# pyannote/pyannote-video

Measured on AMD Instinct MI355X. Metric: frames/sec end-to-end detect->embed->cluster, 1080p@25fps, higher is better.
Workload: dtype f32 (detector scores, embedder) / f64 (tracker, clustering) / u8 frames; an f16 screening pass with a proven error bound decides which windows the detector's exact f32 chain is evaluated for -- results identical to dense f32 scoring (`dense_scoring`)

## Files before the change

pyannote-video_amd/csrc/api.hip:

```cpp
#include "pvf_internal.h"
#include <algorithm>
#include <cmath>
#include <cstdlib>
#include <string>
#include <thread>

#define API_BEGIN try {
#define API_END                                                        \
    return 0;                                                          \
    }                                                                  \
    catch (const std::exception& e) { pvf_set_error(e.what()); return -1; } \
    catch (...) { pvf_set_error("unknown error"); return -2; }

#define ENTER(c, h)                                                \
    Ctx* c = pvf_ctx(h);                                           \
    std::lock_guard<std::recursive_mutex> _api_lock(c->api_mu);    \
    HIP_CHECK(hipSetDevice(c->device))
#define ENTER_DET(c, h)                                            \
    Ctx* c = pvf_ctx(h);                                           \
    std::lock_guard<std::recursive_mutex> _det_lock(c->det_mu);    \
    HIP_CHECK(hipSetDevice(c->device))
#define ENTER_BOTH(c, h)                                           \
    Ctx* c = pvf_ctx(h);                                           \
    std::lock_guard<std::recursive_mutex> _det_lock(c->det_mu);    \
// ... 829 lines not shown
        const size_t bytes = (size_t)n * 150 * 150 * 3;
        c->s_trk0.ensure(bytes);
        HIP_CHECK(hipMemcpyAsync(c->s_trk0.p, chips, bytes, hipMemcpyHostToDevice, c->stream));
    }
    resnet_debug_stage(c, c->s_trk0.as<uint8_t>(), n, split != 0, &tap, flags);
    for (int i = 0; i < 3; ++i) dims[i] = tap.dims[i];
    API_END
}

extern "C" int32_t pvf_debug_conv(pvf_handle h, const int32_t geom[18], const float* in, const float* w, const float* bias, const float* gamma,
                                  const float* beta, const float* skip, int32_t split, int32_t force_generic, float* out, int32_t* flags)
{
    API_BEGIN
    ENTER(c, h);
    PVF_REQUIRE(geom, "pvf_debug_conv: bad arguments");
    resnet_debug_conv(c, geom, in, w, bias, gamma, beta, skip, split != 0, force_generic != 0, out, flags);
    API_END
}

extern "C" int32_t pvf_debug_embed_head(pvf_handle h, const float* x, int32_t n, int32_t hw, float* out)
{
    API_BEGIN
    ENTER(c, h);
    resnet_debug_head(c, x, n, hw, out);
    API_END
}

static PairInput table_f64(const double* X) { PairInput in; in.X = X; return in; }
static PairOutput host_full(double* D) { PairOutput o; o.out = D; return o; }

extern "C" int32_t pvf_pair_mean_dist(pvf_handle h, const double* X, int32_t N, int32_t dim, const int32_t* row_start, int32_t T, double* D)
// ... 374 lines not shown
```

pyannote-video_amd/csrc/ctx.hip:

```cpp
#include "pvf_internal.h"
#include "detect_ml.h"
#include <cmath>
#include <fstream>
#include <mutex>
#include <dlfcn.h>

static thread_local std::string g_err;
void pvf_set_error(const char* msg) { g_err = msg ? msg : ""; }
extern "C" const char* pvf_last_error(void) { return g_err.c_str(); }

static std::mutex g_ctx_mu;
static std::unordered_map<uint64_t, std::unique_ptr<Ctx>> g_ctxs;
static uint64_t g_next_ctx = 0x1000;

Ctx* pvf_ctx(pvf_handle h)
{
    std::lock_guard<std::mutex> lk(g_ctx_mu);
    auto it = g_ctxs.find(h);
    if (it == g_ctxs.end()) throw PvfError("unknown context handle");
    return it->second.get();
}

std::map<std::string, Tensor> pvf_read_container(const char* path)
{
// ... 143 lines not shown
{
    auto m = pvf_read_model(path, 2);
    EmbedModel& e = c->emb;
    e.chip_size = need(m, "emb.meta").i32()[0];
    e.chip_padding = need(m, "emb.padding").f64()[0];
    PVF_REQUIRE(e.chip_size == 150, "embedder: 150x150 chips expected");
    const Tensor& ms = need(m, "emb.mean_shape");
    PVF_REQUIRE(ms.numel() == 102, "emb.mean_shape must be 51x2");
    e.mean_shape.assign(ms.f32(), ms.f32() + 102);
    const Tensor& blob = need(m, "emb.blob");
    const float* p = blob.f32();
    const float* end = p + blob.numel();
    for (ConvLayer& L : e.convs) {
        if (L.d_frag) { (void)hipFree(L.d_frag); L.d_frag = nullptr; }
        if (L.d_wsplit) { (void)hipFree(L.d_wsplit); L.d_wsplit = nullptr; }
    }
    e.convs.clear();
    if (e.d_stem) { (void)hipFree(e.d_stem); e.d_stem = nullptr; }
    auto add_conv = [&](int cin, int cout, int k, int stride, int pad) {
        ConvLayer L{cin, cout, k, stride, pad, nullptr, nullptr, nullptr, nullptr, nullptr};
        const size_t nw = (size_t)cout * cin * k * k;
        PVF_REQUIRE(p + nw + 3 * (size_t)cout <= end, "emb.blob too short");
        conv_layer_upload(L, p, p + nw, p + nw + cout, p + nw + 2 * (size_t)cout);
        p += nw + 3 * (size_t)cout;
        e.convs.push_back(L);
    };
    add_conv(3, 32, 7, 2, 0);
    for (int u = 0; u < 14; ++u) {
        const int cin = UNITS[u][0], n = UNITS[u][1], down = UNITS[u][2];
        add_conv(cin, n, 3, down ? 2 : 1, down ? 0 : 1);
        add_conv(n, n, 3, 1, 1);
    }
// ... 385 lines not shown
```

pyannote-video_amd/csrc/pvf_internal.h:

```cpp
#pragma once
#include <hip/hip_runtime.h>
#include <cstdint>
#include <cstdio>
#include <cstring>
#include <deque>
#include <map>
#include <atomic>
#include <memory>
#include <mutex>
#include <stdexcept>
#include <string>
#include <unordered_map>
#include <vector>
#include "../../include/pvface.h"
#include "scratch_layout.h"
#include "chip_plan.h"

#define PVF_FHOG_STRIDE 32

struct CandOverflow : PvfError { int needed; explicit CandOverflow(int n) : PvfError("detector: candidate buffer overflow"), needed(n) {} };
struct ScreenRetry : PvfError { ScreenRetry() : PvfError("detector: screening pass gave up") {} };

#define HIP_CHECK(expr)                                                                              \
    do {                                                                                             \
// ... 115 lines not shown
    int32_t* d_idx1 = nullptr;
    int32_t* d_idx2 = nullptr;
    float* d_thresh = nullptr;
    float* d_leaves = nullptr;
};

struct ConvLayer {
    int cin, cout, k, stride, pad;
    float* d_w;
    float* d_bias;
    float* d_gamma;
    float* d_beta;
    float* d_frag = nullptr;
    int w_exp = 0;
    uint32_t* d_wsplit = nullptr;
};

struct EmbedModel {
    bool loaded = false;
    int chip_size = 150;
    double chip_padding = 0.25;
    std::vector<float> mean_shape;
    std::vector<ConvLayer> convs;
    float* d_fc = nullptr;
    float* d_blob = nullptr;
    float* d_stem = nullptr;
};

struct TrackerTables {
    bool set = false;
    double* d_mask64 = nullptr;
    double* d_mask_scale = nullptr;
    double* d_tw64 = nullptr;
    double* d_tw32 = nullptr;
    double alpha_pow_m16 = 0, ln_alpha = 0;
};

struct Tracker {
    double* d_state = nullptr;
    int* share = nullptr;
    double pos[4] = {0, 0, 0, 0};
// ... 170 lines not shown
void jitter_embed_dev(Ctx* c, const uint8_t* d_chips, int n, int J, uint64_t seed, float* out);
void ert_run(Ctx* c, const std::vector<Frame>& frames, const pvf_rect_i32* boxes, int n, int32_t* pts, float* shape = nullptr);
void face_chip_details(const EmbedModel& m, const int32_t* pts68, ChipDetails* out);
void dlib_mean_face_shape(float* out );
void resnet_forward(Ctx* c, const uint8_t* d_chips, int n, float* h_out);
struct ChipSource { const uint8_t* host; const pvf_handle* frames; const int32_t* pts; };
const EmbedModel& faces_geometry();
void faces_make_chips(Ctx* c, const pvf_handle* frames, const int32_t* pts, int m, uint8_t* d_chips);
void faces_source_round(Ctx* c, const ChipSource& src, int i0, int m, uint8_t* d_chips);
void conv_layer_upload(ConvLayer& L, const float* w, const float* bias, const float* gamma, const float* beta);
void conv_layer_free(ConvLayer& L);
#define EMB_STAGES 30
struct EmbedTap { int stage; float* h_out; int dims[3]; };
void resnet_debug_stage(Ctx* c, const uint8_t* d_chips, int n, bool split, EmbedTap* tap, int* h_flags);
void resnet_debug_conv(Ctx* c, const int32_t* geom, const float* in, const float* w, const float* bias, const float* gamma, const float* beta,
                       const float* skip, bool split, bool force_generic, float* out, int32_t* flags);
void resnet_debug_head(Ctx* c, const float* x, int n, int hw, float* out);
void dsst_start_many(Ctx* c, const std::vector<Tracker*>& t, const std::vector<Frame>& f, const double* boxes);
void dsst_clone_many(Ctx* c, const std::vector<Tracker*>& src, const std::vector<Tracker*>& dst);
double* tracker_state_alloc(Ctx* c);
void shot_dfd(Ctx* c, const std::vector<Frame>& frames, int ow, int oh, const float* tables22, double* dfd, uint8_t* gray_out, float* flow_out);
std::vector<int> orb_level_quota();
void orb_extract(Ctx* c, const std::vector<Frame>& frames, int ow, int oh, int cap, int32_t* counts, float* kp_out, uint8_t* desc_out);
void orb_match_counts(Ctx* c, const uint8_t* desc, const int32_t* nrows, int n_sets, int cap, const int32_t* pairs, int64_t n_pairs, int32_t* out);
void dsst_update_many(Ctx* c, const std::vector<Tracker*>& t, const std::vector<Frame>& f, double* psr, double* boxes_out, int mode = 0);
void overlap_matrix_host(const double* a, int na, const double* b, int nb, double ratio, double* out);
void munkres_host(const double* cost, int n, int32_t* row_to_col);
struct PairInput {
    const double* X = nullptr;
    const float* emb = nullptr; int64_t emb_stride = 0; int n_src = 0; const int32_t* order = nullptr; int decimals = -1; bool emb_on_device = false;
};
// ... 14 lines not shown
```

pyannote-video_amd/csrc/resnet.hip:

```cpp
#include "pvf_internal.h"
#include <cmath>
#include <cstdlib>
#include <cstring>
#include <vector>

typedef float f32x4 __attribute__((ext_vector_type(4)));
typedef uint32_t u32x4 __attribute__((ext_vector_type(4)));
typedef float f32x16 __attribute__((ext_vector_type(16)));
typedef _Float16 f16x8 __attribute__((ext_vector_type(8)));
typedef _Float16 f16x4 __attribute__((ext_vector_type(4)));
typedef uint32_t u32x2 __attribute__((ext_vector_type(2)));

void face_chip_details(const EmbedModel& m, const int32_t* pts, ChipDetails* out)
{
    const double size = m.chip_size, padding = m.chip_padding;
    double fx[51], fy[51], tx[51], ty[51];
    int n = 0;
    for (int i = 17; i < 68; ++i) {
        if ((55 <= i && i <= 59) || (65 <= i && i <= 67)) continue;
        if (17 <= i && i <= 26) continue;
        fx[n] = ((padding + (double)m.mean_shape[2 * (i - 17)]) / (2 * padding + 1)) * size;
        fy[n] = ((padding + (double)m.mean_shape[2 * (i - 17) + 1]) / (2 * padding + 1)) * size;
        tx[n] = pts[2 * i]; ty[n] = pts[2 * i + 1];
        ++n;
// ... 18 lines not shown
    out->cs = ca / scale; out->sn = cb / scale;
    out->rows = m.chip_size; out->cols = m.chip_size;
}

struct ConvArgs {
    const float* in; int B, H, W, Cin;
    const float* w; int K;
    const float* frag;
    const float* bias; const float* gamma; const float* beta;
    float* out; int OH, OW, Cout;
    int AH, AW;
    int ksz, stride, pad;
    int skip_mode;
    const float* skip; int XH, XW, XC, SH, SW;
    const uint32_t* wsplit; float out_scale; int* flags;
};


__device__ __forceinline__ int small_div(int x, int d, float rd)
{
    int q = (int)((float)x * rd);
    const int r = x - q * d;
    q += (r >= d) ? 1 : 0;
    q -= (r < 0) ? 1 : 0;
    return q;
}

template <int WM, int WN>
__device__ __forceinline__ void conv_epilogue(const ConvArgs& a, float* smem, const f32x16& acc0, const f32x16& acc1, long M, long m0, int n0,
                                              int rel0, int b_first, int hw, float r_hw, float r_ow, int wave, int lane)
// ... 311 lines not shown
        }
    }
    const float bs = bias[li], g = gamma[li], bt = beta[li];
    float* o = out + ((size_t)face * OW + oy0) * OW * 32 + li;
#pragma unroll
    for (int t = 0; t < 3; ++t)
#pragma unroll
        for (int reg = 0; reg < 16; ++reg) {
            const int m = (wave * 3 + t) * 32 + (reg & 3) + 8 * (reg >> 2) + 4 * kh;
            float v = (acc[t][reg] + bs) * g + bt;
            v = v < 0.0f ? 0.0f : v;
            o[(size_t)m * 32] = v;
        }
}

#define C32_ROWS 7
#define C32_TILE_FLOATS (9 * 37 * 33)
__global__ void __launch_bounds__(64) conv_frag_k(const float* __restrict__ w, int Kpad, float* __restrict__ frag)
{
    const int s = blockIdx.x, l = threadIdx.x;
    frag[s * 64 + l] = w[(size_t)(l & 31) * Kpad + 2 * s + (l >> 5)];
}

__global__ void __launch_bounds__(256) conv3x3_c32_k(const float* __restrict__ in, const float* __restrict__ frag, const float* __restrict__ bias,
                                                     const float* __restrict__ gamma, const float* __restrict__ beta, const float* __restrict__ skip,
                                                     float* __restrict__ out, int n_items)
{
    constexpr int HW = 35, TW = 37, PITCH = 33, NP = 144;
    constexpr int NSLOT = 9 * TW * 8, PER = (NSLOT + 255) / 256;
    extern __shared__ __attribute__((aligned(16))) float smem_c32[];
// ... 90 lines not shown
            for (int t = 0; t < 2; ++t)
#pragma unroll
                for (int reg = 0; reg < 16; ++reg) {
                    const float y = ((acc[t][reg] + bs) * g + bt) + sk[t][reg];
                    x[t][reg] = y < 0.0f ? 0.0f : y;
                }
        } else {
#pragma unroll
            for (int t = 0; t < 2; ++t)
#pragma unroll
                for (int reg = 0; reg < 16; ++reg) {
                    const float y = (acc[t][reg] + bs) * g + bt;
                    x[t][reg] = y < 0.0f ? 0.0f : y;
                }
        }
#pragma unroll
        for (int t = 0; t < 2; ++t)
#pragma unroll
            for (int reg = 0; reg < 16; ++reg)
                __builtin_amdgcn_raw_buffer_store_b32(__builtin_bit_cast(uint32_t, x[t][reg]), ro, e_off[t][reg], 0, 0);
        __syncthreads();
        item = next;
    }
}

__global__ void __launch_bounds__(256) maxpool3s2_k(const float* __restrict__ in, int B, int H, int W, int C, float* __restrict__ out, int OH, int OW)
{
    const size_t i = (size_t)blockIdx.x * blockDim.x + threadIdx.x;
    const size_t total = (size_t)B * OH * OW * C;
    if (i >= total) return;
// ... 26 lines not shown
    }
}

static bool conv_is_c32(const ConvArgs& a)
{
    return a.Cin == 32 && a.Cout == 32 && a.H == 35 && a.W == 35 && a.OH == 35 && a.OW == 35 && a.AH == 35 && a.AW == 35 && a.ksz == 3 &&
           a.stride == 1 && a.pad == 1 && a.skip_mode != 2;
}

static void launch_conv(Ctx* c, const ConvArgs& a)
{
    const long M = (long)a.B * a.OH * a.OW;
    PVF_REQUIRE(a.Cin % 32 == 0, "conv: input channels must be a multiple of 32 (the 3-channel first layer has a kernel of its own: stem_conv_k)");
    PVF_REQUIRE(a.OH * a.OW < (1 << 21) && a.Cout % 32 == 0, "conv: output map too large for the kernel's index arithmetic / Cout not a multiple of 32");
    auto tile = [&](auto exact, auto split, dim3 grid) { hipLaunchKernelGGL((a.wsplit ? split : exact), grid, dim3(256), 0, c->stream, a); };
    if (a.frag && conv_is_c32(a)) {
        static std::atomic<uint64_t> attr_set{0};
        const size_t lds = (size_t)(C32_TILE_FLOATS + 144 * 64) * sizeof(float);
        const uint64_t bit = 1ull << (c->device & 63);
        if (!(attr_set.load() & bit)) {
            HIP_CHECK(hipFuncSetAttribute(reinterpret_cast<const void*>(conv3x3_c32_k), hipFuncAttributeMaxDynamicSharedMemorySize, (int)lds));
            attr_set.fetch_or(bit);
        }
        const int items = a.B * (35 / C32_ROWS);
        hipLaunchKernelGGL(conv3x3_c32_k, dim3((unsigned)std::min(items, 2 * c->n_cu)), dim3(256), lds, c->stream, a.in, a.frag, a.bias, a.gamma, a.beta,
                           a.skip_mode == 1 ? a.skip : nullptr, a.out, items);
    } else if (a.Cout == 32) {
        tile(conv_tile_k<4, 1, ConvExact>, conv_tile_k<4, 1, ConvSplit>, dim3((unsigned)((M + 255) / 256), 1));
    } else {
        PVF_REQUIRE(a.Cout % 64 == 0, "conv: Cout must be 32 or a multiple of 64");
        tile(conv_tile_k<2, 2, ConvExact>, conv_tile_k<2, 2, ConvSplit>, dim3((unsigned)((M + 127) / 128), a.Cout / 64));
// ... 19 lines not shown
        HIP_CHECK(hipMemcpy(d, src, count * sizeof(float), hipMemcpyHostToDevice));
        return d;
    };
    L.d_w = up(wt.data(), wt.size());
    float wmax = 0.0f;
    for (float v : wt) wmax = std::max(wmax, std::fabs(v));
    int ex = 0;
    if (wmax > 0.0f && std::isfinite(wmax)) { std::frexp(wmax, &ex); L.w_exp = 15 - ex; }
    L.d_bias = up(bias, cout);
    L.d_gamma = up(gamma, cout);
    L.d_beta = up(beta, cout);
}

void conv_layer_free(ConvLayer& L)
{
    for (void* p : {(void*)L.d_w, (void*)L.d_bias, (void*)L.d_gamma, (void*)L.d_beta, (void*)L.d_frag, (void*)L.d_wsplit})
        if (p) (void)hipFree(p);
    L.d_w = L.d_bias = L.d_gamma = L.d_beta = L.d_frag = nullptr;
    L.d_wsplit = nullptr;
}

static void conv_bind_weights(Ctx* c, ConvLayer& L, bool split, bool generic, int* flags, ConvArgs& a)
{
    a.w = L.d_w; a.K = L.k * L.k * L.cin; a.bias = L.d_bias; a.gamma = L.d_gamma; a.beta = L.d_beta;
    a.frag = nullptr; a.wsplit = nullptr; a.out_scale = 0.0f; a.flags = nullptr;
    if (!generic && L.cin == 32 && L.cout == 32 && L.k == 3) {
        if (!conv_is_c32(a)) return;
        if (!L.d_frag) {
            HIP_CHECK(hipMalloc(&L.d_frag, 144 * 64 * sizeof(float)));
            hipLaunchKernelGGL(conv_frag_k, dim3(144), dim3(64), 0, c->stream, L.d_w, 288, L.d_frag);
        }
        a.frag = L.d_frag;
        return;
    }
    if (!split) return;
    if (!L.d_wsplit) {
        const int Kpad = (L.k * L.k * L.cin + 31) / 32 * 32;
        const int total = L.cout * Kpad;
        HIP_CHECK(hipMalloc(&L.d_wsplit, (size_t)total * 2 * sizeof(_Float16)));
        hipLaunchKernelGGL(conv_wsplit_k, dim3((unsigned)((total + 255) / 256)), dim3(256), 0, c->stream, L.d_w, total, L.w_exp,
                           reinterpret_cast<_Float16*>(L.d_wsplit));
    }
// ... 92 lines not shown
    c->s_act1.ensure(big * sizeof(float));
    c->s_act2.ensure((size_t)cap * hp * hp * 32 * sizeof(float) + (size_t)cap * 128 * sizeof(float));
    PVF_REQUIRE(!tap || n <= MAXB, "embedder stage access: at most 4096 faces");
    auto tapped = [&](int stage, const float* d, int B, int H, int W, int C) {
        if (tap && tap->stage == stage && tap->h_out)
            HIP_CHECK(hipMemcpyAsync(tap->h_out, d, (size_t)B * H * W * C * sizeof(float), hipMemcpyDeviceToHost, c->stream));
    };
    for (int b0 = 0; b0 < n; b0 += MAXB) {
        const int B = std::min(MAXB, n - b0);
        ProfScope ps(c, "conv");
        float* x = c->s_act0.as<float>();
        float* y = c->s_act1.as<float>();
        float* z = c->s_act2.as<float>();
        const ConvLayer& L0 = e.convs[0];
        PVF_REQUIRE(S == 150 && L0.cout == 32 && L0.k == 7 && h1 == 72, "stem kernel: 150 x 150 chips, 7 x 7 stride 2, 32 channels");
        if (!c->emb.d_stem) {
            HIP_CHECK(hipMalloc(&c->emb.d_stem, STEM_NP * 64 * sizeof(float)));
            hipLaunchKernelGGL(stem_frag_k, dim3(STEM_NP), dim3(64), 0, c->stream, L0.d_w, c->emb.d_stem);
        }
        hipLaunchKernelGGL(stem_conv_k, dim3(h1 / STEM_ROWS, B), dim3(192), 0, c->stream, d_chips + (size_t)b0 * S * S * 3, B, c->emb.d_stem,
                           L0.d_bias, L0.d_gamma, L0.d_beta, y);
        tapped(0, y, B, h1, h1, 32);
        ConvArgs a;
        const size_t npool = (size_t)B * hp * hp * 32;
        hipLaunchKernelGGL(maxpool3s2_k, dim3((unsigned)((npool + 255) / 256)), dim3(256), 0, c->stream, y, B, h1, h1, 32, z, hp, hp);
        tapped(1, z, B, hp, hp, 32);
        float* cur = z; float* t1 = x; float* t2 = y;
        int H = hp;
        int* flags = nullptr;
        if (split) {
            flags = c->s_emb_flags.as<int>();
            HIP_CHECK(hipMemsetAsync(flags, 0, (size_t)B * sizeof(int), c->stream));
        }
        for (int u = 0; u < 14; ++u) {
            const int cin = UN[u][0], nn = UN[u][1], down = UN[u][2];
            ConvLayer& La = c->emb.convs[1 + 2 * u];
            ConvLayer& Lb = c->emb.convs[2 + 2 * u];
            const int stride = down ? 2 : 1, pad = down ? 0 : 1;
            const auto [ah, sh, oh] = unit_dims(u, H);
            memset(&a, 0, sizeof a);
            a.in = cur; a.B = B; a.H = H; a.W = H; a.Cin = cin;
            a.out = t1; a.OH = ah; a.OW = ah; a.Cout = nn; a.AH = ah; a.AW = ah; a.ksz = 3; a.stride = stride; a.pad = pad; a.skip_mode = 0;
            conv_bind_weights(c, La, split, false, flags, a);
            launch_conv(c, a);
            tapped(2 + 2 * u, t1, B, ah, ah, nn);
            memset(&a, 0, sizeof a);
            a.in = t1; a.B = B; a.H = ah; a.W = ah; a.Cin = nn;
            a.out = t2; a.OH = oh; a.OW = oh; a.Cout = nn; a.AH = ah; a.AW = ah; a.ksz = 3; a.stride = 1; a.pad = 1;
            a.skip_mode = down ? 2 : 1; a.skip = cur; a.XH = H; a.XW = H; a.XC = cin; a.SH = sh; a.SW = sh;
            conv_bind_weights(c, Lb, split, false, flags, a);
            launch_conv(c, a);
            tapped(3 + 2 * u, t2, B, oh, oh, nn);
            float* old = cur; cur = t2; t2 = old;
            H = oh;
        }
        float* d_out = reinterpret_cast<float*>(c->s_act2.as<uint8_t>() + (size_t)cap * hp * hp * 32 * sizeof(float));
        hipLaunchKernelGGL(head_k, dim3(B), dim3(256), 0, c->stream, cur, H * H, e.d_fc, d_out);
        HIP_CHECK(hipGetLastError());
        HIP_CHECK(hipMemcpyAsync(h_out + (size_t)b0 * 128, d_out, (size_t)B * 128 * sizeof(float), hipMemcpyDeviceToHost, c->stream));
        if (split) HIP_CHECK(hipMemcpyAsync(h_flags + b0, flags, (size_t)B * sizeof(int), hipMemcpyDeviceToHost, c->stream));
    }
    HIP_CHECK(hipStreamSynchronize(c->stream));
}

void resnet_forward(Ctx* c, const uint8_t* d_chips, int n, float* h_out)
// ... 43 lines not shown
struct Scoped {
    void* p = nullptr;
    explicit Scoped(size_t bytes) { HIP_CHECK(hipMalloc(&p, bytes ? bytes : 4)); }
    ~Scoped() { if (p) (void)hipFree(p); }
    Scoped(const Scoped&) = delete;
    Scoped& operator=(const Scoped&) = delete;
};
struct ScopedLayer {
    ConvLayer L{};
    ~ScopedLayer() { conv_layer_free(L); }
};
struct Drain { Ctx* c; ~Drain() { (void)hipStreamSynchronize(c->stream); } };
}

void resnet_debug_conv(Ctx* c, const int32_t* g, const float* in, const float* w, const float* bias, const float* gamma, const float* beta,
                       const float* skip, bool split, bool force_generic, float* out, int32_t* flags)
{
    ConvArgs a;
    memset(&a, 0, sizeof a);
    a.B = g[0]; a.H = g[1]; a.W = g[2]; a.Cin = g[3]; a.OH = g[4]; a.OW = g[5]; a.Cout = g[6]; a.AH = g[7]; a.AW = g[8];
    a.ksz = g[9]; a.stride = g[10]; a.pad = g[11]; a.skip_mode = g[12]; a.XH = g[13]; a.XW = g[14]; a.XC = g[15]; a.SH = g[16]; a.SW = g[17];
    PVF_REQUIRE(in && w && bias && gamma && beta && out, "pvf_debug_conv: null tensor");
    PVF_REQUIRE(a.B > 0 && a.H > 0 && a.W > 0 && a.Cin > 0 && a.OH > 0 && a.OW > 0 && a.Cout > 0 && a.ksz > 0 && a.ksz <= 7 && a.stride > 0 && a.pad >= 0,
                "pvf_debug_conv: bad dimensions");
    PVF_REQUIRE(a.AH > 0 && a.AW > 0 && a.AH <= a.OH && a.AW <= a.OW, "pvf_debug_conv: the convolution's extent must lie inside the output map");
    PVF_REQUIRE(a.skip_mode >= 0 && a.skip_mode <= 2 && (a.skip_mode == 0 || skip), "pvf_debug_conv: skip_mode must be 0..2, with a skip tensor for 1 and 2");
    const size_t n_in = (size_t)a.B * a.H * a.W * a.Cin, n_out = (size_t)a.B * a.OH * a.OW * a.Cout;
    size_t n_skip = 0;
    if (a.skip_mode == 1) n_skip = n_out;
    if (a.skip_mode == 2) {
        PVF_REQUIRE(a.XH > 0 && a.XW > 0 && a.XC > 0 && a.SH >= 0 && a.SW >= 0 && 2 * a.SH <= a.XH && 2 * a.SW <= a.XW,
                    "pvf_debug_conv: the averaged skip map must lie inside the skip tensor");
        n_skip = (size_t)a.B * a.XH * a.XW * a.XC;
    }
    PVF_REQUIRE(n_in < (1u << 30) && n_out < (1u << 30) && n_skip < (1u << 30), "pvf_debug_conv: tensor too large");
    ScopedLayer sl;
    sl.L.cin = a.Cin; sl.L.cout = a.Cout; sl.L.k = a.ksz; sl.L.stride = a.stride; sl.L.pad = a.pad;
// ... 39 lines not shown
```

pyannote-video_amd/pyannote_video_amd/runtime.py:

```python
import contextlib
import ctypes as C
import threading
import itertools
import operator
import numpy as np
from . import _lib
from ._lib import check, ptr, handles
from . import models as _models
from .y4m import YuvFrame, chroma_shape


class DeviceFrame(object):
    __slots__ = ("ctx", "handle", "height", "width", "keep", "transient", "__weakref__")

    def __init__(self, ctx, handle, height, width, keep=None, transient=False):
        self.ctx, self.handle, self.height, self.width, self.keep = ctx, handle, height, width, keep
        self.transient = transient

    @property
    def shape(self):
        return (self.height, self.width, 3)

    def release(self):
        if self.handle is not None and self.ctx._h is not None:
# ... 789 lines not shown
        if skip_mode == 2:
            _, xh, xw, xc = skip.shape
            sh, sw = xh // 2, xw // 2
        oh, ow = out_hw if out_hw is not None else (max(ah, sh), max(aw, sw))
        if skip_mode == 1 and skip.shape != (B, oh, ow, cout):
            raise ValueError("debug_conv: the skip tensor must have the output's shape")
        if skip_mode == 2 and skip.shape[0] != B:
            raise ValueError("debug_conv: one skip map per face")
        par = [np.ascontiguousarray(v, np.float32).reshape(-1) for v in (bias, gamma, beta)]
        if any(v.size != cout for v in par):
            raise ValueError("debug_conv: bias, gamma and beta have one value per output channel")
        geom = np.array([B, H, W, cin, oh, ow, cout, ah, aw, k, stride, pad, skip_mode, xh, xw, xc, sh, sw], np.int32)
        out = np.zeros((B, max(oh, 0), max(ow, 0), cout), np.float32)
        flags = np.zeros(B, np.int32)
        check(self._l.pvf_debug_conv(self._h, ptr(geom), ptr(x), ptr(w), ptr(par[0]), ptr(par[1]), ptr(par[2]),
                                     ptr(skip) if skip is not None else None, 1 if split else 0, 1 if force_generic else 0, ptr(out), ptr(flags)))
        return out, flags

    def embed_head(self, x):
        x = np.ascontiguousarray(x, np.float32)
        n, hw, ch = x.shape
        if ch != 256:
            raise ValueError("embed_head: 256 channels")
        out = np.zeros((n, 128), np.float32)
        check(self._l.pvf_debug_embed_head(self._h, ptr(x), n, hw, ptr(out)))
        return out

    def shot_dfd(self, frames, width, height, tables, want_gray=False, want_flow=False):
        n = len(frames)
        t = np.ascontiguousarray(tables, np.float32)
        if t.shape != (22,):
# ... 284 lines not shown
```

Measured before the change: 4870.

## Add split-f16 MFMA kernels for embedder stem and 32-channel 3x3 convs

Adds new embedder kernels that represent activations and weights as hi/lo f16 pairs and accumulate with 32x32x16 f16 MFMA. They cover the 7x7 stem and the 32-channel 3x3 residual convs, using persistent blocks, prefetch of the next item and LDS-resident weight fragments. The split path now also covers the stem, and the flags buffer is set up before the stem runs. This is meant to replace slower exact-f32 or older split convolution code with higher-throughput matrix-core work. It adds precision-split bookkeeping with overflow flags and more LDS use per block.

```diff
diff --git a/pyannote-video_amd/csrc/api.hip b/pyannote-video_amd/csrc/api.hip
--- a/pyannote-video_amd/csrc/api.hip
+++ b/pyannote-video_amd/csrc/api.hip
@@ -867,7 +867,7 @@
     API_BEGIN
     ENTER(c, h);
     PVF_REQUIRE(geom, "pvf_debug_conv: bad arguments");
-    resnet_debug_conv(c, geom, in, w, bias, gamma, beta, skip, split != 0, force_generic != 0, out, flags);
+    resnet_debug_conv(c, geom, in, w, bias, gamma, beta, skip, split, force_generic != 0, out, flags);
     API_END
 }
 
diff --git a/pyannote-video_amd/csrc/ctx.hip b/pyannote-video_amd/csrc/ctx.hip
--- a/pyannote-video_amd/csrc/ctx.hip
+++ b/pyannote-video_amd/csrc/ctx.hip
@@ -181,8 +181,10 @@
     for (ConvLayer& L : e.convs) {
         if (L.d_frag) { (void)hipFree(L.d_frag); L.d_frag = nullptr; }
         if (L.d_wsplit) { (void)hipFree(L.d_wsplit); L.d_wsplit = nullptr; }
+        if (L.d_fsplit) { (void)hipFree(L.d_fsplit); L.d_fsplit = nullptr; }
     }
     e.convs.clear();
+    if (e.d_stem_split) { (void)hipFree(e.d_stem_split); e.d_stem_split = nullptr; }
     if (e.d_stem) { (void)hipFree(e.d_stem); e.d_stem = nullptr; }
     auto add_conv = [&](int cin, int cout, int k, int stride, int pad) {
         ConvLayer L{cin, cout, k, stride, pad, nullptr, nullptr, nullptr, nullptr, nullptr};
diff --git a/pyannote-video_amd/csrc/pvf_internal.h b/pyannote-video_amd/csrc/pvf_internal.h
--- a/pyannote-video_amd/csrc/pvf_internal.h
+++ b/pyannote-video_amd/csrc/pvf_internal.h
@@ -153,6 +153,7 @@
     float* d_frag = nullptr;
     int w_exp = 0;
     uint32_t* d_wsplit = nullptr;
+    uint32_t* d_fsplit = nullptr;
 };
 
 struct EmbedModel {
@@ -164,6 +165,7 @@
     float* d_fc = nullptr;
     float* d_blob = nullptr;
     float* d_stem = nullptr;
+    uint32_t* d_stem_split = nullptr;
 };
 
 struct TrackerTables {
@@ -364,7 +366,7 @@
 struct EmbedTap { int stage; float* h_out; int dims[3]; };
 void resnet_debug_stage(Ctx* c, const uint8_t* d_chips, int n, bool split, EmbedTap* tap, int* h_flags);
 void resnet_debug_conv(Ctx* c, const int32_t* geom, const float* in, const float* w, const float* bias, const float* gamma, const float* beta,
-                       const float* skip, bool split, bool force_generic, float* out, int32_t* flags);
+                       const float* skip, int split, bool force_generic, float* out, int32_t* flags);
 void resnet_debug_head(Ctx* c, const float* x, int n, int hw, float* out);
 void dsst_start_many(Ctx* c, const std::vector<Tracker*>& t, const std::vector<Frame>& f, const double* boxes);
 void dsst_clone_many(Ctx* c, const std::vector<Tracker*>& src, const std::vector<Tracker*>& dst);
diff --git a/pyannote-video_amd/csrc/resnet.hip b/pyannote-video_amd/csrc/resnet.hip
--- a/pyannote-video_amd/csrc/resnet.hip
+++ b/pyannote-video_amd/csrc/resnet.hip
@@ -56,6 +56,7 @@
     int skip_mode;
     const float* skip; int XH, XW, XC, SH, SW;
     const uint32_t* wsplit; float out_scale; int* flags;
+    const uint32_t* fsplit;
 };
 
 
@@ -397,6 +398,148 @@
         }
 }
 
+#define STEMS_STEPS 14
+#define STEMS_PLANE 5872
+#define STEMS_FRAG_DW (STEMS_STEPS * 2 * 64 * 4)
+#define STEMS_LDS_BYTES (4 * STEMS_PLANE * 2 + STEMS_FRAG_DW * 4)
+#define STEMS_ITEMS_PER_FACE (72 / STEM_ROWS)
+__global__ void __launch_bounds__(64) stem_frag_split_k(const float* __restrict__ w, int w_exp, _Float16* __restrict__ frag)
+{
+    const int S = blockIdx.x, l = threadIdx.x, r = S >> 1;
+    _Float16* hi = frag + ((size_t)(2 * S) * 64 + l) * 8;
+    _Float16* lo = hi + 64 * 8;
+    for (int j = 0; j < 8; ++j) {
+        const int t = 16 * (S & 1) + 8 * (l >> 5) + j;
+        const float v = (t < 21) ? ldexpf(w[(size_t)(l & 31) * 224 + (r * 7 + t / 3) * 4 + t % 3], w_exp) : 0.0f;
+        hi[j] = (_Float16)v;
+        lo[j] = (_Float16)(v - (float)hi[j]);
+    }
+}
+
+__global__ void __launch_bounds__(192) stem_split_k(const uint8_t* __restrict__ chips, const uint32_t* __restrict__ frag, const float* __restrict__ bias,
+                                                    const float* __restrict__ gamma, const float* __restrict__ beta, float out_scale,
+                                                    float* __restrict__ out, int n_items)
+{
+    constexpr int S = 150, OW = 72, ROWV = S * 3, PER = (STEM_IN_DW + 191) / 192, NI = STEMS_ITEMS_PER_FACE;
+    constexpr int RSRC_FLAGS = 0x00020000, OOB = (int)0x80000000;
+    constexpr int CHIP_BYTES = S * S * 3, ITEM_BYTES = STEM_ROWS * OW * 32 * 4;
+    extern __shared__ __attribute__((aligned(16))) uint32_t smem_stems[];
+    _Float16* P = reinterpret_cast<_Float16*>(smem_stems);
+    uint32_t* Pd = smem_stems;
+    uint32_t* Bf = smem_stems + 2 * STEMS_PLANE;
+    const int tid = threadIdx.x, lane = tid & 63, wave = tid >> 6;
+    const int li = lane & 31, kh = lane >> 5;
+    {
+        const u32x4* f4 = reinterpret_cast<const u32x4*>(frag);
+        u32x4* b4 = reinterpret_cast<u32x4*>(Bf);
+        for (int i = tid; i < STEMS_FRAG_DW / 4; i += 192) b4[i] = f4[i];
+        if (tid < 18) {
+            P[2 * STEMS_PLANE + 5854 + tid] = (_Float16)0.0f;
+            P[3 * STEMS_PLANE + 5854 + tid] = (_Float16)0.0f;
+            if (tid >= 2) { P[5854 + tid] = (_Float16)0.0f; P[STEMS_PLANE + 5854 + tid] = (_Float16)0.0f; }
+        }
+    }
+    const float bs = bias[li], g = gamma[li], bt = beta[li];
+    int off_e[3], off_o[3];
+#pragma unroll
+    for (int t = 0; t < 3; ++t) {
+        const int m = (wave * 3 + t) * 32 + li;
+        const int oy = m / OW, ox = m - oy * OW;
+        const int idx = (2 * oy) * ROWV + 6 * ox + 8 * kh;
+        const int plain = idx, moved = 2 * STEMS_PLANE + idx - 2;
+        off_e[t] = (ox & 1) ? moved : plain;
+        off_o[t] = (ox & 1) ? plain : moved;
+    }
+    const uint32_t* bl = Bf + lane * 4;
+    const float M[3] = {122.782f, 117.001f, 104.298f};
+    const float m4[4] = {M[tid % 3], M[(tid + 1) % 3], M[(tid + 2) % 3], M[tid % 3]};
+    int d_off[PER];
+#pragma unroll
+    for (int j = 0; j < PER; ++j) d_off[j] = (tid + j * 192 < STEM_IN_DW) ? 4 * (tid + j * 192) : OOB;
+    uint32_t v[PER];
+    auto request = [&](int item) {
+        const int face = item / NI, first = 2 * (item - face * NI) * STEM_ROWS * ROWV;
+        const __amdgpu_buffer_rsrc_t rc = __builtin_amdgcn_make_buffer_rsrc((void*)(chips + (size_t)face * CHIP_BYTES), 0, CHIP_BYTES, RSRC_FLAGS);
+#pragma unroll
+        for (int j = 0; j < PER; ++j) v[j] = __builtin_amdgcn_raw_buffer_load_b32(rc, (int)((unsigned)first + (unsigned)d_off[j]), 0, 0);
+    };
+    int item = blockIdx.x;
+    if (item < n_items) request(item);
+    while (item < n_items) {
+#pragma unroll
+        for (int j = 0; j < PER; ++j) {
+            const int d = tid + j * 192;
+            if (d < STEM_IN_DW) {
+                f32x4 x;
+#pragma unroll
+                for (int k = 0; k < 4; ++k) x[k] = (float)((v[j] >> (8 * k)) & 255u) - m4[k];
+                const f16x4 hi = __builtin_convertvector(x, f16x4), lo = __builtin_convertvector(x - __builtin_convertvector(hi, f32x4), f16x4);
+                const u32x2 h2 = __builtin_bit_cast(u32x2, hi), l2 = __builtin_bit_cast(u32x2, lo);
+                *reinterpret_cast<u32x2*>(Pd + 2 * d) = h2;
+                *reinterpret_cast<u32x2*>(Pd + STEMS_PLANE / 2 + 2 * d) = l2;
+                uint32_t* q = Pd + STEMS_PLANE + 2 * d - 1;
+                if (d > 0) { q[0] = h2.x; q[STEMS_PLANE / 2] = l2.x; }
+                q[1] = h2.y; q[STEMS_PLANE / 2 + 1] = l2.y;
+            }
+        }
+        __syncthreads();
+        const int next = item + gridDim.x;
+        if (next < n_items) request(next);
+        f32x16 acc[3];
+#pragma unroll
+        for (int t = 0; t < 3; ++t)
+#pragma unroll
+            for (int i = 0; i < 16; ++i) acc[t][i] = 0.0f;
+        f16x8 fa[2][6], fb[2][2];
+        auto read16 = [&](int half) {
+            typedef const volatile __attribute__((address_space(3))) u32x2 lds_u32x2;
+            lds_u32x2* p = (lds_u32x2*)(P + half);
+            const u32x2 a = p[0], b = p[1];
+            const u32x4 r = {a.x, a.y, b.x, b.y};
+            return __builtin_bit_cast(f16x8, r);
+        };
+        auto fetch = [&](int K, f16x8* A, f16x8* Bv) {
+            const int r = K >> 1, c = r * ROWV + 16 * (K & 1);
+            Bv[0] = *reinterpret_cast<const f16x8*>(bl + (2 * K) * 256);
+            Bv[1] = *reinterpret_cast<const f16x8*>(bl + (2 * K + 1) * 256);
+#pragma unroll
+            for (int t = 0; t < 3; ++t) {
+                const int o = ((r & 1) ? off_o[t] : off_e[t]) + c;
+                A[2 * t] = read16(o);
+                A[2 * t + 1] = read16(o + STEMS_PLANE);
+            }
+        };
+        fetch(0, fa[0], fb[0]);
+#pragma unroll
+        for (int K = 0; K < STEMS_STEPS; ++K) {
+            if (K + 1 < STEMS_STEPS) fetch(K + 1, fa[(K + 1) & 1], fb[(K + 1) & 1]);
+            __builtin_amdgcn_sched_barrier(0);
+            const f16x8 *A = fa[K & 1], *Bv = fb[K & 1];
+#pragma unroll
+            for (int t = 0; t < 3; ++t) acc[t] = __builtin_amdgcn_mfma_f32_32x32x16_f16(A[2 * t], Bv[0], acc[t], 0, 0, 0);
+#pragma unroll
+            for (int t = 0; t < 3; ++t) acc[t] = __builtin_amdgcn_mfma_f32_32x32x16_f16(A[2 * t], Bv[1], acc[t], 0, 0, 0);
+#pragma unroll
+            for (int t = 0; t < 3; ++t) acc[t] = __builtin_amdgcn_mfma_f32_32x32x16_f16(A[2 * t + 1], Bv[0], acc[t], 0, 0, 0);
+        }
+        const int face = item / NI, oy0 = (item - face * NI) * STEM_ROWS;
+        const __amdgpu_buffer_rsrc_t ro = __builtin_amdgcn_make_buffer_rsrc((void*)(out + ((size_t)face * OW + oy0) * OW * 32), 0, ITEM_BYTES, RSRC_FLAGS);
+        const int e0 = ((wave * 96 + 4 * kh) * 32 + li) * 4;
+#pragma unroll
+        for (int t = 0; t < 3; ++t) {
+            acc[t] *= out_scale;
+#pragma unroll
+            for (int reg = 0; reg < 16; ++reg) {
+                float y = (acc[t][reg] + bs) * g + bt;
+                y = y < 0.0f ? 0.0f : y;
+                __builtin_amdgcn_raw_buffer_store_b32(__builtin_bit_cast(uint32_t, y), ro, e0 + ((t * 32 + (reg & 3) + 8 * (reg >> 2)) * 32) * 4, 0, 0);
+            }
+        }
+        __syncthreads();
+        item = next;
+    }
+}
+
 #define C32_ROWS 7
 #define C32_TILE_FLOATS (9 * 37 * 33)
 __global__ void __launch_bounds__(64) conv_frag_k(const float* __restrict__ w, int Kpad, float* __restrict__ frag)
@@ -517,6 +660,164 @@
                     x[t][reg] = y < 0.0f ? 0.0f : y;
                 }
         }
+#pragma unroll
+        for (int t = 0; t < 2; ++t)
+#pragma unroll
+            for (int reg = 0; reg < 16; ++reg)
+                __builtin_amdgcn_raw_buffer_store_b32(__builtin_bit_cast(uint32_t, x[t][reg]), ro, e_off[t][reg], 0, 0);
+        __syncthreads();
+        item = next;
+    }
+}
+
+#ifndef C32S_ROWS
+#define C32S_ROWS 7
+#endif
+#define C32S_BLOCKS_PER_CU (C32S_ROWS == 7 ? 1 : 2)
+#define C32S_STEPS 18
+#define C32S_FRAG_DW (C32S_STEPS * 2 * 64 * 4)
+template <int ROWS> constexpr int c32s_lds_bytes() { return ((ROWS + 2) * 37 * 36 + C32S_FRAG_DW) * 4; }
+
+__global__ void __launch_bounds__(64) conv_frag_split_k(const float* __restrict__ w, int Kpad, int w_exp, _Float16* __restrict__ frag)
+{
+    const int S = blockIdx.x, l = threadIdx.x;
+    const float* src = w + (size_t)(l & 31) * Kpad + 16 * S + 8 * (l >> 5);
+    _Float16* hi = frag + ((size_t)(2 * S) * 64 + l) * 8;
+    _Float16* lo = hi + 64 * 8;
+    for (int j = 0; j < 8; ++j) {
+        const float v = ldexpf(src[j], w_exp);
+        hi[j] = (_Float16)v;
+        lo[j] = (_Float16)(v - (float)hi[j]);
+    }
+}
+
+template <int ROWS>
+__global__ void __launch_bounds__(256) conv3x3_c32_split_k(const float* __restrict__ in, const uint32_t* __restrict__ frag, const float* __restrict__ bias,
+                                                           const float* __restrict__ gamma, const float* __restrict__ beta, const float* __restrict__ skip,
+                                                           float* __restrict__ out, float out_scale, int* __restrict__ flags, int n_items)
+{
+    constexpr int HW = 35, TW = 37, PITCH = 36, TR = ROWS + 2, NB = HW / ROWS;
+    static_assert(HW % ROWS == 0, "bands of equal height");
+    constexpr int NSLOT = TR * TW * 8, PER = (NSLOT + 255) / 256;
+    constexpr int NPIX = ROWS * HW, NT = (NPIX + 31) / 32;
+    static_assert(NT > 4 && NT <= 8, "one or two tiles per wave");
+    constexpr int RSRC_FLAGS = 0x00020000, OOB = (int)0x80000000;
+    constexpr int FACE_BYTES = HW * HW * 32 * 4, ROW_BYTES = HW * 32 * 4, BAND_BYTES = ROWS * ROW_BYTES;
+    extern __shared__ __attribute__((aligned(16))) uint32_t smem_c32s[];
+    uint32_t* T = smem_c32s;
+    uint32_t* Bf = smem_c32s + TR * TW * PITCH;
+    const int tid = threadIdx.x, lane = tid & 63, wave = tid >> 6;
+    const int li = lane & 31, kh = lane >> 5;
+    {
+        const u32x4* f4 = reinterpret_cast<const u32x4*>(frag);
+        u32x4* b4 = reinterpret_cast<u32x4*>(Bf);
+        for (int i = tid; i < C32S_FRAG_DW / 4; i += 256) b4[i] = f4[i];
+    }
+    const float bs = bias[li], g = gamma[li], bt = beta[li];
+    const bool two = NT == 8 || wave + 4 < NT;
+    const uint32_t* base[2];
+#pragma unroll
+    for (int t = 0; t < 2; ++t) {
+        int m = (wave + 4 * t) * 32 + li;
+        if (m >= NPIX) m = 0;
+        const int oy = m / HW, ox = m - oy * HW;
+        base[t] = T + (oy * TW + ox) * PITCH + 4 * kh;
+    }
+    const uint32_t* bl = Bf + lane * 4;
+    int s_off[PER];
+#pragma unroll
+    for (int j = 0; j < PER; ++j) {
+        const int i = tid + j * 256;
+        const int c4 = i & 7, px = i >> 3;
+        const int ry = px / TW, cx = px - ry * TW;
+        s_off[j] = ((i < NSLOT) && ((unsigned)(cx - 1) < (unsigned)HW)) ? ((ry * HW + (cx - 1)) * 32 + 4 * c4) * 4 : OOB;
+    }
+    u32x4 v[PER];
+    float sk[2][16];
+    auto request = [&](int item) {
+        const int face = item / NB, band = item - face * NB;
+        const __amdgpu_buffer_rsrc_t ri = __builtin_amdgcn_make_buffer_rsrc((void*)(in + (size_t)face * (FACE_BYTES / 4)), 0, FACE_BYTES, RSRC_FLAGS);
+        const int row0 = (band * ROWS - 1) * ROW_BYTES;
+#pragma unroll
+        for (int j = 0; j < PER; ++j) v[j] = __builtin_amdgcn_raw_buffer_load_b128(ri, (int)((unsigned)row0 + (unsigned)s_off[j]), 0, 0);
+    };
+    int e_off[2][16];
+#pragma unroll
+    for (int t = 0; t < 2; ++t)
+#pragma unroll
+        for (int reg = 0; reg < 16; ++reg) e_off[t][reg] = (((wave + 4 * t) * 32 + (reg & 3) + 8 * (reg >> 2) + 4 * kh) * 32 + li) * 4;
+    auto request_skip = [&](int item) {
+        const int face = item / NB, oy0 = (item - face * NB) * ROWS;
+        const __amdgpu_buffer_rsrc_t rk = __builtin_amdgcn_make_buffer_rsrc((void*)(skip + ((size_t)face * HW + oy0) * HW * 32), 0, BAND_BYTES, RSRC_FLAGS);
+#pragma unroll
+        for (int t = 0; t < 2; ++t)
+#pragma unroll
+            for (int reg = 0; reg < 16; ++reg) sk[t][reg] = __builtin_bit_cast(float, __builtin_amdgcn_raw_buffer_load_b32(rk, e_off[t][reg], 0, 0));
+    };
+    int item = blockIdx.x;
+    if (item < n_items) request(item);
+    while (item < n_items) {
+        bool ok = true;
+#pragma unroll
+        for (int j = 0; j < PER; ++j) {
+            const int i = tid + j * 256;
+            if (i < NSLOT) ok &= ConvSplit::park_a(T + (i >> 3) * PITCH, i & 7, v[j]);
+        }
+        if (!ok) flags[item / NB] = 1;
+        __syncthreads();
+        const int next = item + gridDim.x;
+        if (next < n_items) request(next);
+        if (skip) request_skip(item);
+        f32x16 acc[2];
+#pragma unroll
+        for (int t = 0; t < 2; ++t)
+#pragma unroll
+            for (int i = 0; i < 16; ++i) acc[t][i] = 0.0f;
+        f16x8 fa[2][4], fb[2][2];
+        auto fetch = [&](int S, f16x8* A, f16x8* B) {
+            const int tap = S >> 1, r = tap / 3, q = tap - r * 3;
+            const int off = (r * TW + q) * PITCH + 8 * (S & 1);
+            B[0] = *reinterpret_cast<const f16x8*>(bl + (2 * S) * 256);
+            B[1] = *reinterpret_cast<const f16x8*>(bl + (2 * S + 1) * 256);
+            A[0] = *reinterpret_cast<const f16x8*>(base[0] + off);
+            A[1] = *reinterpret_cast<const f16x8*>(base[0] + off + 16);
+            if (two) {
+                A[2] = *reinterpret_cast<const f16x8*>(base[1] + off);
+                A[3] = *reinterpret_cast<const f16x8*>(base[1] + off + 16);
+            }
+        };
+        fetch(0, fa[0], fb[0]);
+#pragma unroll
+        for (int S = 0; S < C32S_STEPS; ++S) {
+            if (S + 1 < C32S_STEPS) fetch(S + 1, fa[(S + 1) & 1], fb[(S + 1) & 1]);
+            __builtin_amdgcn_sched_barrier(0);
+            const f16x8 *A = fa[S & 1], *B = fb[S & 1];
+            if (two) {
+                acc[0] = __builtin_amdgcn_mfma_f32_32x32x16_f16(A[0], B[0], acc[0], 0, 0, 0);
+                acc[1] = __builtin_amdgcn_mfma_f32_32x32x16_f16(A[2], B[0], acc[1], 0, 0, 0);
+                acc[0] = __builtin_amdgcn_mfma_f32_32x32x16_f16(A[0], B[1], acc[0], 0, 0, 0);
+                acc[1] = __builtin_amdgcn_mfma_f32_32x32x16_f16(A[2], B[1], acc[1], 0, 0, 0);
+                acc[0] = __builtin_amdgcn_mfma_f32_32x32x16_f16(A[1], B[0], acc[0], 0, 0, 0);
+                acc[1] = __builtin_amdgcn_mfma_f32_32x32x16_f16(A[3], B[0], acc[1], 0, 0, 0);
+            } else {
+                acc[0] = __builtin_amdgcn_mfma_f32_32x32x16_f16(A[0], B[0], acc[0], 0, 0, 0);
+                acc[0] = __builtin_amdgcn_mfma_f32_32x32x16_f16(A[0], B[1], acc[0], 0, 0, 0);
+                acc[0] = __builtin_amdgcn_mfma_f32_32x32x16_f16(A[1], B[0], acc[0], 0, 0, 0);
+            }
+        }
+        acc[0] *= out_scale;
+        acc[1] *= out_scale;
+        const int face = item / NB, oy0 = (item - face * NB) * ROWS;
+        const __amdgpu_buffer_rsrc_t ro = __builtin_amdgcn_make_buffer_rsrc((void*)(out + ((size_t)face * HW + oy0) * HW * 32), 0, BAND_BYTES, RSRC_FLAGS);
+        float x[2][16];
+#pragma unroll
+        for (int t = 0; t < 2; ++t)
+#pragma unroll
+            for (int reg = 0; reg < 16; ++reg) {
+                float y = (acc[t][reg] + bs) * g + bt;
+                if (skip) y += sk[t][reg];
+                x[t][reg] = y < 0.0f ? 0.0f : y;
+            }
 #pragma unroll
         for (int t = 0; t < 2; ++t)
 #pragma unroll
@@ -573,7 +874,18 @@
     PVF_REQUIRE(a.Cin % 32 == 0, "conv: input channels must be a multiple of 32 (the 3-channel first layer has a kernel of its own: stem_conv_k)");
     PVF_REQUIRE(a.OH * a.OW < (1 << 21) && a.Cout % 32 == 0, "conv: output map too large for the kernel's index arithmetic / Cout not a multiple of 32");
     auto tile = [&](auto exact, auto split, dim3 grid) { hipLaunchKernelGGL((a.wsplit ? split : exact), grid, dim3(256), 0, c->stream, a); };
-    if (a.frag && conv_is_c32(a)) {
+    if (a.fsplit && conv_is_c32(a)) {
+        static std::atomic<uint64_t> attr_set{0};
+        constexpr int lds = c32s_lds_bytes<C32S_ROWS>();
+        const uint64_t bit = 1ull << (c->device & 63);
+        if (!(attr_set.load() & bit)) {
+            HIP_CHECK(hipFuncSetAttribute(reinterpret_cast<const void*>(conv3x3_c32_split_k<C32S_ROWS>), hipFuncAttributeMaxDynamicSharedMemorySize, lds));
+            attr_set.fetch_or(bit);
+        }
+        const int items = a.B * (35 / C32S_ROWS);
+        hipLaunchKernelGGL(conv3x3_c32_split_k<C32S_ROWS>, dim3((unsigned)std::min(items, C32S_BLOCKS_PER_CU * c->n_cu)), dim3(256), lds, c->stream, a.in,
+                           a.fsplit, a.bias, a.gamma, a.beta, a.skip_mode == 1 ? a.skip : nullptr, a.out, a.out_scale, a.flags, items);
+    } else if (a.frag && conv_is_c32(a)) {
         static std::atomic<uint64_t> attr_set{0};
         const size_t lds = (size_t)(C32_TILE_FLOATS + 144 * 64) * sizeof(float);
         const uint64_t bit = 1ull << (c->device & 63);
@@ -623,18 +935,28 @@
 
 void conv_layer_free(ConvLayer& L)
 {
-    for (void* p : {(void*)L.d_w, (void*)L.d_bias, (void*)L.d_gamma, (void*)L.d_beta, (void*)L.d_frag, (void*)L.d_wsplit})
+    for (void* p : {(void*)L.d_w, (void*)L.d_bias, (void*)L.d_gamma, (void*)L.d_beta, (void*)L.d_frag, (void*)L.d_wsplit, (void*)L.d_fsplit})
         if (p) (void)hipFree(p);
     L.d_w = L.d_bias = L.d_gamma = L.d_beta = L.d_frag = nullptr;
-    L.d_wsplit = nullptr;
-}
-
-static void conv_bind_weights(Ctx* c, ConvLayer& L, bool split, bool generic, int* flags, ConvArgs& a)
+    L.d_wsplit = L.d_fsplit = nullptr;
+}
+
+static void conv_bind_weights(Ctx* c, ConvLayer& L, int split, bool generic, int* flags, ConvArgs& a)
 {
     a.w = L.d_w; a.K = L.k * L.k * L.cin; a.bias = L.d_bias; a.gamma = L.d_gamma; a.beta = L.d_beta;
-    a.frag = nullptr; a.wsplit = nullptr; a.out_scale = 0.0f; a.flags = nullptr;
+    a.frag = nullptr; a.wsplit = nullptr; a.fsplit = nullptr; a.out_scale = 0.0f; a.flags = nullptr;
     if (!generic && L.cin == 32 && L.cout == 32 && L.k == 3) {
         if (!conv_is_c32(a)) return;
+        if (split == 2) {
+            if (!L.d_fsplit) {
+                HIP_CHECK(hipMalloc(&L.d_fsplit, C32S_FRAG_DW * sizeof(uint32_t)));
+                hipLaunchKernelGGL(conv_frag_split_k, dim3(C32S_STEPS), dim3(64), 0, c->stream, L.d_w, 288, L.w_exp, reinterpret_cast<_Float16*>(L.d_fsplit));
+            }
+            a.fsplit = L.d_fsplit;
+            a.out_scale = std::ldexp(1.0f, -(EMB_A_SCALE_EXP + L.w_exp));
+            a.flags = flags;
+            return;
+        }
         if (!L.d_frag) {
             HIP_CHECK(hipMalloc(&L.d_frag, 144 * 64 * sizeof(float)));
             hipLaunchKernelGGL(conv_frag_k, dim3(144), dim3(64), 0, c->stream, L.d_w, 288, L.d_frag);
@@ -757,12 +1079,34 @@
         float* z = c->s_act2.as<float>();
         const ConvLayer& L0 = e.convs[0];
         PVF_REQUIRE(S == 150 && L0.cout == 32 && L0.k == 7 && h1 == 72, "stem kernel: 150 x 150 chips, 7 x 7 stride 2, 32 channels");
-        if (!c->emb.d_stem) {
+        if (!split && !c->emb.d_stem) {
             HIP_CHECK(hipMalloc(&c->emb.d_stem, STEM_NP * 64 * sizeof(float)));
             hipLaunchKernelGGL(stem_frag_k, dim3(STEM_NP), dim3(64), 0, c->stream, L0.d_w, c->emb.d_stem);
         }
-        hipLaunchKernelGGL(stem_conv_k, dim3(h1 / STEM_ROWS, B), dim3(192), 0, c->stream, d_chips + (size_t)b0 * S * S * 3, B, c->emb.d_stem,
-                           L0.d_bias, L0.d_gamma, L0.d_beta, y);
+        int* flags = nullptr;
+        if (split) {
+            flags = c->s_emb_flags.as<int>();
+            HIP_CHECK(hipMemsetAsync(flags, 0, (size_t)B * sizeof(int), c->stream));
+        }
+        if (split) {
+            if (!c->emb.d_stem_split) {
+                HIP_CHECK(hipMalloc(&c->emb.d_stem_split, STEMS_FRAG_DW * sizeof(uint32_t)));
+                hipLaunchKernelGGL(stem_frag_split_k, dim3(STEMS_STEPS), dim3(64), 0, c->stream, L0.d_w, L0.w_exp, reinterpret_cast<_Float16*>(c->emb.d_stem_split));
+            }
+            static std::atomic<uint64_t> attr_set{0};
+            const uint64_t bit = 1ull << (c->device & 63);
+            if (!(attr_set.load() & bit)) {
+                HIP_CHECK(hipFuncSetAttribute(reinterpret_cast<const void*>(stem_split_k), hipFuncAttributeMaxDynamicSharedMemorySize, STEMS_LDS_BYTES));
+                attr_set.fetch_or(bit);
+            }
+            const int items = B * STEMS_ITEMS_PER_FACE;
+            hipLaunchKernelGGL(stem_split_k, dim3((unsigned)std::min(items, 2 * c->n_cu)), dim3(192), STEMS_LDS_BYTES, c->stream,
+                               d_chips + (size_t)b0 * S * S * 3, c->emb.d_stem_split, L0.d_bias, L0.d_gamma, L0.d_beta,
+                               std::ldexp(1.0f, -(EMB_A_SCALE_EXP + L0.w_exp)), y, items);
+        } else {
+            hipLaunchKernelGGL(stem_conv_k, dim3(h1 / STEM_ROWS, B), dim3(192), 0, c->stream, d_chips + (size_t)b0 * S * S * 3, B, c->emb.d_stem,
+                               L0.d_bias, L0.d_gamma, L0.d_beta, y);
+        }
         tapped(0, y, B, h1, h1, 32);
         ConvArgs a;
         const size_t npool = (size_t)B * hp * hp * 32;
@@ -770,11 +1114,6 @@
         tapped(1, z, B, hp, hp, 32);
         float* cur = z; float* t1 = x; float* t2 = y;
         int H = hp;
-        int* flags = nullptr;
-        if (split) {
-            flags = c->s_emb_flags.as<int>();
-            HIP_CHECK(hipMemsetAsync(flags, 0, (size_t)B * sizeof(int), c->stream));
-        }
         for (int u = 0; u < 14; ++u) {
             const int cin = UN[u][0], nn = UN[u][1], down = UN[u][2];
             ConvLayer& La = c->emb.convs[1 + 2 * u];
@@ -784,14 +1123,14 @@
             memset(&a, 0, sizeof a);
             a.in = cur; a.B = B; a.H = H; a.W = H; a.Cin = cin;
             a.out = t1; a.OH = ah; a.OW = ah; a.Cout = nn; a.AH = ah; a.AW = ah; a.ksz = 3; a.stride = stride; a.pad = pad; a.skip_mode = 0;
-            conv_bind_weights(c, La, split, false, flags, a);
+            conv_bind_weights(c, La, split ? 2 : 0, false, flags, a);
             launch_conv(c, a);
             tapped(2 + 2 * u, t1, B, ah, ah, nn);
             memset(&a, 0, sizeof a);
             a.in = t1; a.B = B; a.H = ah; a.W = ah; a.Cin = nn;
             a.out = t2; a.OH = oh; a.OW = oh; a.Cout = nn; a.AH = ah; a.AW = ah; a.ksz = 3; a.stride = 1; a.pad = 1;
             a.skip_mode = down ? 2 : 1; a.skip = cur; a.XH = H; a.XW = H; a.XC = cin; a.SH = sh; a.SW = sh;
-            conv_bind_weights(c, Lb, split, false, flags, a);
+            conv_bind_weights(c, Lb, split ? 2 : 0, false, flags, a);
             launch_conv(c, a);
             tapped(3 + 2 * u, t2, B, oh, oh, nn);
             float* old = cur; cur = t2; t2 = old;
@@ -865,13 +1204,14 @@
 }
 
 void resnet_debug_conv(Ctx* c, const int32_t* g, const float* in, const float* w, const float* bias, const float* gamma, const float* beta,
-                       const float* skip, bool split, bool force_generic, float* out, int32_t* flags)
+                       const float* skip, int split, bool force_generic, float* out, int32_t* flags)
 {
     ConvArgs a;
     memset(&a, 0, sizeof a);
     a.B = g[0]; a.H = g[1]; a.W = g[2]; a.Cin = g[3]; a.OH = g[4]; a.OW = g[5]; a.Cout = g[6]; a.AH = g[7]; a.AW = g[8];
     a.ksz = g[9]; a.stride = g[10]; a.pad = g[11]; a.skip_mode = g[12]; a.XH = g[13]; a.XW = g[14]; a.XC = g[15]; a.SH = g[16]; a.SW = g[17];
     PVF_REQUIRE(in && w && bias && gamma && beta && out, "pvf_debug_conv: null tensor");
+    PVF_REQUIRE(split >= 0 && split <= 2, "pvf_debug_conv: split must be 0 (exact), 1 or 2");
     PVF_REQUIRE(a.B > 0 && a.H > 0 && a.W > 0 && a.Cin > 0 && a.OH > 0 && a.OW > 0 && a.Cout > 0 && a.ksz > 0 && a.ksz <= 7 && a.stride > 0 && a.pad >= 0,
                 "pvf_debug_conv: bad dimensions");
     PVF_REQUIRE(a.AH > 0 && a.AW > 0 && a.AH <= a.OH && a.AW <= a.OW, "pvf_debug_conv: the convolution's extent must lie inside the output map");
diff --git a/pyannote-video_amd/pyannote_video_amd/runtime.py b/pyannote-video_amd/pyannote_video_amd/runtime.py
--- a/pyannote-video_amd/pyannote_video_amd/runtime.py
+++ b/pyannote-video_amd/pyannote_video_amd/runtime.py
@@ -827,7 +827,7 @@
         out = np.zeros((B, max(oh, 0), max(ow, 0), cout), np.float32)
         flags = np.zeros(B, np.int32)
         check(self._l.pvf_debug_conv(self._h, ptr(geom), ptr(x), ptr(w), ptr(par[0]), ptr(par[1]), ptr(par[2]),
-                                     ptr(skip) if skip is not None else None, 1 if split else 0, 1 if force_generic else 0, ptr(out), ptr(flags)))
+                                     ptr(skip) if skip is not None else None, int(split), 1 if force_generic else 0, ptr(out), ptr(flags)))
         return out, flags
 
     def embed_head(self, x):
```

After: 4985, median of 5. 1.02x the previous value.
